# Negai-98/LDT

Measured on AMD Instinct MI355X. Metric: shapes/sec (2048-pt, 1000-step SDE sample), higher is better.
Workload: dtype bf16

## Files before the change

### ldt_amd/csrc/attn_tile.h

```cpp
#pragma once
#include "kernels.h"

template <int DH>
struct AttnLaneOffs {
    int k0;
    int v[DH / 32];
    __device__ __forceinline__ void init(int lane) {
        constexpr int ROWB = DH * 2;
        const int r = lane & 31, hh = lane >> 5;
        const int swk = (DH == 64) ? ((r >> 1) & 7) : ((r >> 2) & 3);
        k0 = r * ROWB + ((hh ^ swk) << 4);
        const int tg = lane >> 4, ti = lane & 15, tq = ti >> 2, tp = ti & 3;
        const int v_row_off = 4 * (tg >> 1) + tq;
        const int v_chunk = (tg & 1) * 2 + (tp >> 1);
        const int v_byte = (tp & 1) * 8;
        const int swv = (DH == 64) ? (((v_row_off >> 1) & 1) << 2) : 0;
#pragma unroll
        for (int d = 0; d < DH / 32; ++d) v[d] = v_row_off * ROWB + (((d * 4 + v_chunk) ^ swv) << 4) + v_byte;
    }
};

#define ATT_THR 6.0f
#ifndef ATT_SCALAR_SOFTMAX
#define ATT_SCALAR_SOFTMAX 0
#endif
template <int DH>
__device__ __forceinline__ void attn_block(const char* Kt, const char* Vt, const int kt, const bf16x8 (&qf)[DH / 16], f32x16 (&oacc)[DH / 32],
                                           float& m_run, float& l_run, int kv0, int Nk, int hh, float c,
                                           const AttnLaneOffs<DH>& lo) {
    constexpr int ROWB = DH * 2, ND = DH / 32, NS = DH / 16;
    {
        f32x16 sacc;
#pragma unroll
        for (int i = 0; i < 16; ++i) sacc[i] = 0.f;
#pragma unroll
        for (int s = 0; s < NS; ++s) {
            const bf16x8 kf = *reinterpret_cast<const bf16x8*>(Kt + kt * 32 * ROWB + (lo.k0 ^ (s << 5)));
            sacc = __builtin_amdgcn_mfma_f32_32x32x16_bf16(kf, qf[s], sacc, 0, 0, 0);
        }
        if (kv0 + kt * 32 + 32 > Nk) {
#pragma unroll
            for (int i = 0; i < 16; ++i) {
                const int key = kv0 + kt * 32 + (i & 3) + 8 * (i >> 2) + 4 * hh;
                sacc[i] = (key < Nk) ? sacc[i] : -INFINITY;
            }
        }
        float mx = __builtin_fmaxf(sacc[0], sacc[1]);
#pragma unroll
        for (int i = 2; i < 16; i += 2) mx = __builtin_fmaxf(__builtin_fmaxf(mx, sacc[i]), sacc[i + 1]);
        mx = fmaxf(mx, __shfl_xor(mx, 32, 64));
        if (__builtin_amdgcn_ballot_w64((mx - m_run) * c > ATT_THR) != 0) {
            const float m_new = fmaxf(m_run, mx);
            const float alpha = __builtin_amdgcn_exp2f((m_run - m_new) * c);
            l_run *= alpha;
            m_run = m_new;
            const f32x2 a2 = {alpha, alpha};
#pragma unroll
            for (int d = 0; d < ND; ++d)
#pragma unroll
                for (int i = 0; i < 16; i += 2) {
                    f32x2 o = {oacc[d][i], oacc[d][i + 1]};
                    o *= a2;
                    oacc[d][i] = o[0]; oacc[d][i + 1] = o[1];
                }
        }
        const f32x2 c2 = {c, c}, nmc2 = {-m_run * c, -m_run * c};
        f32x2 ps2 = {0.f, 0.f};
        bf16x8 pf[2];
#pragma unroll
        for (int i = 0; i < 16; i += 2) {
            const f32x2 sv = {sacc[i], sacc[i + 1]};
            const f32x2 e = sv * c2 + nmc2;
            f32x2 pv;
            pv[0] = __builtin_amdgcn_exp2f(e[0]);
            pv[1] = __builtin_amdgcn_exp2f(e[1]);
            ps2 += pv;
            pf[i >> 3][i & 7] = (bf16_t)pv[0];
            pf[i >> 3][(i & 7) + 1] = (bf16_t)pv[1];
        }
        l_run += ps2[0] + ps2[1];
#pragma unroll
        for (int s2 = 0; s2 < 2; ++s2)
#pragma unroll
            for (int d = 0; d < ND; ++d) {
                const char* base = Vt + (kt * 32 + 16 * s2) * ROWB;
                const bf16x4 v0 = __builtin_amdgcn_ds_read_tr16_b64_v4bf16((__attribute__((address_space(3))) bf16x4*)(base + lo.v[d]));
                const bf16x4 v1 = __builtin_amdgcn_ds_read_tr16_b64_v4bf16((__attribute__((address_space(3))) bf16x4*)(base + 8 * ROWB + lo.v[d]));
                const bf16x8 vf = {v0[0], v0[1], v0[2], v0[3], v1[0], v1[1], v1[2], v1[3]};
                oacc[d] = __builtin_amdgcn_mfma_f32_32x32x16_bf16(vf, pf[s2], oacc[d], 0, 0, 0);
            }
    }
}
template <int DH>
__device__ __forceinline__ void attn_tile(const char* Kt, const char* Vt, const bf16x8 (&qf)[DH / 16], f32x16 (&oacc)[DH / 32],
                                          float& m_run, float& l_run, int kv0, int Nk, int hh, float c,
                                          const AttnLaneOffs<DH>& lo) {
    attn_block<DH>(Kt, Vt, 0, qf, oacc, m_run, l_run, kv0, Nk, hh, c, lo);
    attn_block<DH>(Kt, Vt, 1, qf, oacc, m_run, l_run, kv0, Nk, hh, c, lo);
}

template <int DH>
__device__ __forceinline__ void attn_scores(const char* Kt, const bf16x8 (&qf)[DH / 16], f32x16& s0, f32x16& s1, const AttnLaneOffs<DH>& lo) {
    constexpr int ROWB = DH * 2, NS = DH / 16;
#pragma unroll
    for (int i = 0; i < 16; ++i) { s0[i] = 0.f; s1[i] = 0.f; }
#pragma unroll
    for (int s = 0; s < NS; ++s) {
        const bf16x8 k0 = *reinterpret_cast<const bf16x8*>(Kt + (lo.k0 ^ (s << 5)));
        const bf16x8 k1 = *reinterpret_cast<const bf16x8*>(Kt + 32 * ROWB + (lo.k0 ^ (s << 5)));
        s0 = __builtin_amdgcn_mfma_f32_32x32x16_bf16(k0, qf[s], s0, 0, 0, 0);
        s1 = __builtin_amdgcn_mfma_f32_32x32x16_bf16(k1, qf[s], s1, 0, 0, 0);
    }
}
template <int DH>
__device__ __forceinline__ void attn_softmax_pv(const char* Vt, f32x16& s0, f32x16& s1, f32x16 (&oacc)[DH / 32], float& m_run, float& l_run,
                                                int kv0, int Nk, int hh, float c, const AttnLaneOffs<DH>& lo) {
    constexpr int ROWB = DH * 2, ND = DH / 32;
    if (kv0 + 64 > Nk) {
#pragma unroll
        for (int i = 0; i < 16; ++i) {
            const int key = kv0 + (i & 3) + 8 * (i >> 2) + 4 * hh;
            s0[i] = (key < Nk) ? s0[i] : -INFINITY;
            s1[i] = (key + 32 < Nk) ? s1[i] : -INFINITY;
        }
    }
    float mx = __builtin_fmaxf(s0[0], s1[0]);
#pragma unroll
    for (int i = 1; i < 16; ++i) mx = __builtin_fmaxf(__builtin_fmaxf(mx, s0[i]), s1[i]);
    mx = fmaxf(mx, __shfl_xor(mx, 32, 64));
    if (__builtin_amdgcn_ballot_w64((mx - m_run) * c > ATT_THR) != 0) {
        const float m_new = fmaxf(m_run, mx);
        const float alpha = __builtin_amdgcn_exp2f((m_run - m_new) * c);
        l_run *= alpha;
        m_run = m_new;
        const f32x2 a2 = {alpha, alpha};
#pragma unroll
        for (int d = 0; d < ND; ++d)
#pragma unroll
            for (int i = 0; i < 16; i += 2) {
                f32x2 o = {oacc[d][i], oacc[d][i + 1]};
                o *= a2;
                oacc[d][i] = o[0]; oacc[d][i + 1] = o[1];
            }
    }
    bf16x8 pf[4];
#if ATT_SCALAR_SOFTMAX
    const float nmc = -m_run * c;
    float q0 = 0.f, q1 = 0.f, q2 = 0.f, q3 = 0.f;
#pragma unroll
    for (int i = 0; i < 16; i += 2) {
        float ea0 = __builtin_fmaf(s0[i], c, nmc), ea1 = __builtin_fmaf(s0[i + 1], c, nmc);
        float eb0 = __builtin_fmaf(s1[i], c, nmc), eb1 = __builtin_fmaf(s1[i + 1], c, nmc);
        asm volatile("" : "+v"(ea0), "+v"(ea1), "+v"(eb0), "+v"(eb1));
        const float pa0 = __builtin_amdgcn_exp2f(ea0), pa1 = __builtin_amdgcn_exp2f(ea1);
        const float pb0 = __builtin_amdgcn_exp2f(eb0), pb1 = __builtin_amdgcn_exp2f(eb1);
        q0 += pa0; q1 += pa1; q2 += pb0; q3 += pb1;
        asm volatile("" : "+v"(q0), "+v"(q1), "+v"(q2), "+v"(q3));
        pf[i >> 3][i & 7] = (bf16_t)pa0;       pf[i >> 3][(i & 7) + 1] = (bf16_t)pa1;
        pf[2 + (i >> 3)][i & 7] = (bf16_t)pb0; pf[2 + (i >> 3)][(i & 7) + 1] = (bf16_t)pb1;
    }
    l_run += (q0 + q1) + (q2 + q3);
#else
    const f32x2 c2 = {c, c}, nmc2 = {-m_run * c, -m_run * c};
    f32x2 psa = {0.f, 0.f}, psb = {0.f, 0.f};
#pragma unroll
    for (int i = 0; i < 16; i += 2) {
        const f32x2 ea = (f32x2){s0[i], s0[i + 1]} * c2 + nmc2;
        const f32x2 eb = (f32x2){s1[i], s1[i + 1]} * c2 + nmc2;
        f32x2 pa, pb;
        pa[0] = __builtin_amdgcn_exp2f(ea[0]); pa[1] = __builtin_amdgcn_exp2f(ea[1]);
        pb[0] = __builtin_amdgcn_exp2f(eb[0]); pb[1] = __builtin_amdgcn_exp2f(eb[1]);
        psa += pa; psb += pb;
        pf[i >> 3][i & 7] = (bf16_t)pa[0];       pf[i >> 3][(i & 7) + 1] = (bf16_t)pa[1];
        pf[2 + (i >> 3)][i & 7] = (bf16_t)pb[0]; pf[2 + (i >> 3)][(i & 7) + 1] = (bf16_t)pb[1];
    }
    l_run += (psa[0] + psa[1]) + (psb[0] + psb[1]);
#endif
#pragma unroll
    for (int s2 = 0; s2 < 4; ++s2)
#pragma unroll
        for (int d = 0; d < ND; ++d) {
            const char* base = Vt + 16 * s2 * ROWB;
            const bf16x4 v0 = __builtin_amdgcn_ds_read_tr16_b64_v4bf16((__attribute__((address_space(3))) bf16x4*)(base + lo.v[d]));
            const bf16x4 v1 = __builtin_amdgcn_ds_read_tr16_b64_v4bf16((__attribute__((address_space(3))) bf16x4*)(base + 8 * ROWB + lo.v[d]));
            const bf16x8 vf = {v0[0], v0[1], v0[2], v0[3], v1[0], v1[1], v1[2], v1[3]};
            oacc[d] = __builtin_amdgcn_mfma_f32_32x32x16_bf16(vf, pf[s2], oacc[d], 0, 0, 0);
        }
}

template <int DH>
__device__ __forceinline__ void attn_head_pipelined(const char* Ks, const char* Vs, int ntl, const bf16x8 (&qf)[DH / 16], f32x16 (&oacc)[DH / 32],
                                                    float& m_run, float& l_run, int Nk, int hh, float c, const AttnLaneOffs<DH>& lo) {
    constexpr int TILE = 64 * DH * 2;
    f32x16 sa0, sa1, sb0, sb1;
    attn_scores<DH>(Ks, qf, sa0, sa1, lo);
    int t = 0;
    for (; t + 2 <= ntl; t += 2) {
        attn_scores<DH>(Ks + (t + 1) * TILE, qf, sb0, sb1, lo);
        __builtin_amdgcn_sched_barrier(0);
        attn_softmax_pv<DH>(Vs + t * TILE, sa0, sa1, oacc, m_run, l_run, t * 64, Nk, hh, c, lo);
        __builtin_amdgcn_sched_barrier(0);
        if (t + 2 < ntl) attn_scores<DH>(Ks + (t + 2) * TILE, qf, sa0, sa1, lo);
        __builtin_amdgcn_sched_barrier(0);
        attn_softmax_pv<DH>(Vs + (t + 1) * TILE, sb0, sb1, oacc, m_run, l_run, (t + 1) * 64, Nk, hh, c, lo);
        __builtin_amdgcn_sched_barrier(0);
    }
    if (t < ntl) attn_softmax_pv<DH>(Vs + t * TILE, sa0, sa1, oacc, m_run, l_run, t * 64, Nk, hh, c, lo);
}

template <int DH>
__device__ __forceinline__ void attn_tile_joint(const char* Kt, const char* Vt, const bf16x8 (&qf)[DH / 16], f32x16 (&oacc)[DH / 32],
                                                float& m_run, float& l_run, int kv0, int Nk, int hh, float c,
                                                const AttnLaneOffs<DH>& lo) {
    f32x16 s0, s1;
    attn_scores<DH>(Kt, qf, s0, s1, lo);
    attn_softmax_pv<DH>(Vt, s0, s1, oacc, m_run, l_run, kv0, Nk, hh, c, lo);
}
```

### ldt_amd/csrc/gemm_bf16.hip

```cpp
#include <stdlib.h>

#include <map>
#include <mutex>
#include <tuple>
#include <type_traits>

#include "kernels.h"

#define BK 64

enum { FOLD_NONE = 0, FOLD_PRODUCER = 1, FOLD_CONSUMER = 2 };

template <int ROWS, int NW = 4>
__device__ __forceinline__ void stage_tile(const bf16_t* __restrict__ g, long ld, int row0, int nrows_total,
                                           int k0, char* lds_tile, int wave, int lane) {
#pragma unroll
    for (int p = 0; p < ROWS / (8 * NW); ++p) {
        const int piece = wave * (ROWS / (8 * NW)) + p;
        const int r = piece * 8 + (lane >> 3);
        const int cdst = lane & 7;
        const int csrc = cdst ^ ((r >> 1) & 7);
        int grow = row0 + r;
        grow = grow < nrows_total ? grow : nrows_total - 1;
        const bf16_t* src = g + (long)grow * ld + k0 + csrc * 8;
// ... 543 lines not shown
        auto ktile = [&](auto flags_c) {
            constexpr int FL = decltype(flags_c)::value;
            constexpr bool SKIP = V3_PREISSUE && (FL & KT_FIRST);
            const char* st = smem2 + (gk & 1) * V3_BUF_BYTES;
            char* nb = smem2 + ((gk + 1) & 1) * V3_BUF_BYTES;
            bf16x8 wf[4], xf[4];
            if (!WREG) {
#pragma unroll
                for (int i = 0; i < 4; ++i) wf[i] = *reinterpret_cast<const bf16x8*>(st + wb0 + i * 2048);
            }
#pragma unroll
            for (int i = 0; i < 4; ++i) xf[i] = *reinterpret_cast<const bf16x8*>(st + xb0 + i * 2048);
#if V3_SCHED == 1
            issue_w(nb, 0, 2);
#else
            if (WREG) wload_h1();
            else if (!SKIP) issue_w(nb);
#endif
            if (FL & KT_FOLD_DMA) {
                if (wave < 2 * a.stats_parts) {
                    const float* src = a.stats_in + ((long)(wave >> 1) * a.M + m0 + (wave & 1) * 128) * 2 + lane * 4;
                    __builtin_amdgcn_global_load_lds((const __attribute__((address_space(1))) void*)src,
                                                     (__attribute__((address_space(3))) void*)(stage_reg + V2_STATS_OFF), 16, 0, 0);
                }
                if (wave < 4 && lane < 32) {
                    const float* src = (wave < 2 ? fold_S : fold_C) + n0 + (wave & 1) * 128 + lane * 4;
                    __builtin_amdgcn_global_load_lds((const __attribute__((address_space(1))) void*)src,
                                                     (__attribute__((address_space(3))) void*)(stage_reg + V2_SC_OFF), 16, 0, 0);
                }
            }
            if ((FL & KT_FOLD_FINAL) && wave < 4) v2_fold_finalize(smem2 + V2_RING_BYTES, tid, a.stats_parts, a.K);
            constexpr int P0W = WREG ? (SKIP ? 8 : 4) : SKIP ? 8 : V3_SCHED == 1 ? 2 : 4;
            constexpr bool AFTER_EPI = (FL & KT_FIRST) || (V3_PREISSUE && !WREG && (FL & KT_SECOND));
            if (AFTER_EPI && prev_staged) asm volatile("s_waitcnt vmcnt(%0)" ::"n"(P0W + EPI_VMEM > 63 ? 63 : P0W + EPI_VMEM) : "memory");
            else asm volatile("s_waitcnt vmcnt(%0)" ::"n"(P0W) : "memory");
            V2_BARRIER();
            if (WREG) {
                asm volatile("" : "+v"(w0[0]), "+v"(w0[1]), "+v"(w0[2]), "+v"(w0[3]));
#pragma unroll
                for (int i = 0; i < 4; ++i) wf[i] = __builtin_bit_cast(bf16x8, w0[i]);
            }
            __builtin_amdgcn_s_setprio(1);
#pragma unroll
            for (int ni = 0; ni < 4; ++ni)
#pragma unroll
                for (int mi = 0; mi < 4; ++mi)
                    acc[ni][mi] = __builtin_amdgcn_mfma_f32_16x16x32_bf16(wf[ni], xf[mi], acc[ni][mi], 0, 0, 0);
            __builtin_amdgcn_s_setprio(0);
            V2_BARRIER();
#pragma unroll
            for (int i = 0; i < 4; ++i) xf[i] = *reinterpret_cast<const bf16x8*>(st + xb0 + (4 + i) * 2048);
#if V3_SCHED == 1
            issue_w(nb, 2, 4);
#else
            if (!SKIP) issue_xa(nb);
#endif
            V2_BARRIER();
            __builtin_amdgcn_s_setprio(1);
#pragma unroll
            for (int ni = 0; ni < 4; ++ni)
#pragma unroll
                for (int mi = 0; mi < 4; ++mi)
                    acc[ni][4 + mi] = __builtin_amdgcn_mfma_f32_16x16x32_bf16(wf[ni], xf[mi], acc[ni][4 + mi], 0, 0, 0);
            __builtin_amdgcn_s_setprio(0);
            V2_BARRIER();
            if (!WREG) {
#pragma unroll
                for (int i = 0; i < 4; ++i) wf[i] = *reinterpret_cast<const bf16x8*>(st + wb1 + i * 2048);
            }
#pragma unroll
            for (int i = 0; i < 4; ++i) xf[i] = *reinterpret_cast<const bf16x8*>(st + xb1 + i * 2048);
#if V3_SCHED == 1
            issue_xa(nb);
#else
            if (!SKIP) { issue_xb(nb); advance(); }
#endif
            if (WREG) {
                wload_h0();
                if (SKIP) asm volatile("s_waitcnt vmcnt(4)" ::: "memory");
                else asm volatile("s_waitcnt vmcnt(8)" ::: "memory");
            }
            V2_BARRIER();
            if (WREG) {
                asm volatile("" : "+v"(w1[0]), "+v"(w1[1]), "+v"(w1[2]), "+v"(w1[3]));
#pragma unroll
                for (int i = 0; i < 4; ++i) wf[i] = __builtin_bit_cast(bf16x8, w1[i]);
            }
            __builtin_amdgcn_s_setprio(1);
#pragma unroll
            for (int ni = 0; ni < 4; ++ni)
#pragma unroll
                for (int mi = 0; mi < 4; ++mi)
                    acc[ni][mi] = __builtin_amdgcn_mfma_f32_16x16x32_bf16(wf[ni], xf[mi], acc[ni][mi], 0, 0, 0);
            __builtin_amdgcn_s_setprio(0);
            V2_BARRIER();
#pragma unroll
            for (int i = 0; i < 4; ++i) xf[i] = *reinterpret_cast<const bf16x8*>(st + xb1 + (4 + i) * 2048);
#if V3_SCHED == 1
            issue_xb(nb);
            advance();
#endif
            constexpr int P3W = WREG ? (SKIP ? 4 : 6) : 2;
            if (!WREG && SKIP && prev_staged) asm volatile("s_waitcnt vmcnt(%0)" ::"n"(2 + EPI_VMEM > 63 ? 63 : 2 + EPI_VMEM) : "memory");
            else asm volatile("s_waitcnt vmcnt(%0)" ::"n"(P3W) : "memory");
            V2_BARRIER();
            __builtin_amdgcn_s_setprio(1);
#pragma unroll
            for (int ni = 0; ni < 4; ++ni)
#pragma unroll
                for (int mi = 0; mi < 4; ++mi)
                    acc[ni][4 + mi] = __builtin_amdgcn_mfma_f32_16x16x32_bf16(wf[ni], xf[mi], acc[ni][4 + mi], 0, 0, 0);
            __builtin_amdgcn_s_setprio(0);
            V2_BARRIER();
            ++gk;
        };
#define KTL(f) std::integral_constant<int, (f)>{}
        if (FOLD == FOLD_CONSUMER) {
            ktile(KTL(KT_FIRST)); ktile(KTL(KT_FOLD_DMA | KT_SECOND)); ktile(KTL(KT_PLAIN)); ktile(KTL(KT_FOLD_FINAL));
            for (int kt = 4; kt < nkt; ++kt) ktile(KTL(KT_PLAIN));
        } else {
            ktile(KTL(KT_FIRST)); ktile(KTL(KT_SECOND));
            for (int kt = 2; kt < nkt; ++kt) ktile(KTL(KT_PLAIN));
        }
#undef KTL
        if (grp == 0) V2_BARRIER();

        prev_staged = true;
#if V3_PREISSUE
        if (!XRING) {
            char* pb = smem2 + ((gk + 1) & 1) * V3_BUF_BYTES;
            if (!WREG) issue_w(pb);
            issue_xa(pb); issue_xb(pb); advance();
        }
#endif
        if (XRING) {
            asm volatile("s_waitcnt vmcnt(0)" ::: "memory");
            V2_BARRIER();
            v2_epilogue_staged<EPI, FOLD, 1>(a, acc, m0, n0, grp, wn, lane, lrow, lchk, gate, stage_reg, smem2 + V2_RING_BYTES, ln_scale,
                                                true, g4_pre, sc4_pre, smem2 + wave * 16384);
#if V3_XRING_BREAK
            break;
#else
            if (WREG) break;
#endif
        } else
            v2_epilogue_staged<EPI, FOLD>(a, acc, m0, n0, grp, wn, lane, lrow, lchk, gate, stage_reg, smem2 + V2_RING_BYTES, ln_scale,
                                          it == 0 && (pre_ok || FOLD == FOLD_PRODUCER), g4_pre, sc4_pre);
    }
    asm volatile("s_waitcnt vmcnt(0)" ::: "memory");
}

#include "attn_tile.h"
#define QA_W_ROWS 192
template <int FOLD>
__global__ __launch_bounds__(512) void gemm_qkv_attn256_kernel(const GemmArgs a) {
    static_assert(FOLD == FOLD_NONE || FOLD == FOLD_CONSUMER, "qkv+attention: plain or LN-folded consumer");
    extern __shared__ __attribute__((aligned(16))) char smem2[];
    const int tid = threadIdx.x;
    const int lane = tid & 63;
    const int wave = __builtin_amdgcn_readfirstlane(tid >> 6);
    const int grp = wave >> 2, wn = wave & 3;
    const int lrow = lane & 15, lchk = lane >> 4;
    const int nkt = a.K >> 6;
    const int hidden = a.N / 3, heads = hidden / 64;

    const int tiles_n = heads;
    const int tiles_m = a.M / 256;
    const int tiles = tiles_m * tiles_n;
    const int G = gridDim.x, bid = blockIdx.x;
    const int nx = G < 8 ? G : 8;
    const int xcd = bid % nx, j = bid / nx;
    const int wpx = (G - xcd + nx - 1) / nx;
    const int c_lo = (int)((long)tiles * xcd / nx), c_hi = (int)((long)tiles * (xcd + 1) / nx);
    const int my_tiles = (c_hi - c_lo - j + wpx - 1) / wpx > 0 ? (c_hi - c_lo - j + wpx - 1) / wpx : 0;
    if (my_tiles == 0) return;
    const int gm = a.group_m;
    auto tile_of = [&](int it, int& m0, int& hd) {
        const int id = c_lo + j + it * wpx;
        if (gm <= 1) { m0 = (id / tiles_n) * 256; hd = id % tiles_n; return; }
        const int per = gm * tiles_n, g = id / per, r = id - g * per;
        const int rows = min(gm, tiles_m - g * gm);
        m0 = (g * gm + r % rows) * 256; hd = r / rows;
    };

    int wvo[3], xavo[2], xbvo[2];
    int wds[3], xads[2], xbds[2];
#pragma unroll
    for (int q = 0; q < 3; ++q) {
        const int pj = wave * 3 + q;
        const int r = pj * 8 + (lane >> 3);
        const int gr = (pj >> 3) * hidden + (r & 63);
        wvo[q] = gr * (int)a.ldw * 2 + (((lane & 7) ^ ((r >> 1) & 7)) << 4);
        wds[q] = V3_OPER_BYTES + pj * 1024;
    }
#pragma unroll
    for (int q = 0; q < 2; ++q) {
        const int pj = wave * 2 + q;
        const int r0 = pj < 8 ? pj * 8 : 128 + (pj - 8) * 8;
        const int ra = r0 + (lane >> 3), rb = ra + 64;
        xavo[q] = ra * (int)a.ldx * 2 + (((lane & 7) ^ ((ra >> 1) & 7)) << 4);
        xbvo[q] = rb * (int)a.ldx * 2 + (((lane & 7) ^ ((rb >> 1) & 7)) << 4);
        xads[q] = r0 * 128;
        xbds[q] = (r0 + 64) * 128;
    }
    const char* sxb = nullptr;
    const char* swb = nullptr;
    int s_it = 0, s_kt = 0, s_inc = 128;
    auto seek = [&](int it) {
        int m0, hd;
        tile_of(it, m0, hd);
        sxb = reinterpret_cast<const char*>(a.X + (long)m0 * a.ldx);
        swb = reinterpret_cast<const char*>(a.W + (long)hd * 64 * a.ldw);
    };
    auto advance = [&]() {
        sxb += s_inc; swb += s_inc;
        if (++s_kt == nkt) {
            s_kt = 0;
            if (++s_it < my_tiles) seek(s_it);
            else { sxb -= s_inc; swb -= s_inc; s_inc = 0; s_kt = -0x40000000; }
        }
    };
    int gk = 0;
    auto issue_w = [&](char* buf) {
#pragma unroll
        for (int q = 0; q < 3; ++q)
            __builtin_amdgcn_global_load_lds((const __attribute__((address_space(1))) void*)(swb + wvo[q]),
                                             (__attribute__((address_space(3))) void*)(buf + wds[q]), 16, 0, 0);
    };
    auto issue_xa = [&](char* buf) {
#pragma unroll
        for (int q = 0; q < 2; ++q)
            __builtin_amdgcn_global_load_lds((const __attribute__((address_space(1))) void*)(sxb + xavo[q]),
                                             (__attribute__((address_space(3))) void*)(buf + xads[q]), 16, 0, 0);
    };
    auto issue_xb = [&](char* buf) {
#pragma unroll
        for (int q = 0; q < 2; ++q)
            __builtin_amdgcn_global_load_lds((const __attribute__((address_space(1))) void*)(sxb + xbvo[q]),
                                             (__attribute__((address_space(3))) void*)(buf + xbds[q]), 16, 0, 0);
    };
    seek(0);
    const int step = ((FOLD != FOLD_NONE) && a.step_ptr) ? *a.step_ptr : 0;
    const float* fold_S = (FOLD == FOLD_CONSUMER) ? a.fold_S + (long)step * a.fold_step_stride : nullptr;
    const float* fold_C = (FOLD == FOLD_CONSUMER) ? a.fold_C + (long)step * a.fold_step_stride : nullptr;

    issue_w(smem2); issue_xa(smem2); issue_xb(smem2); advance();
    asm volatile("s_waitcnt vmcnt(2)" ::: "memory");
    V2_BARRIER();

    const int sw = (lrow >> 1) & 7;
    const int xrb = (grp * 128 + lrow) * 128, wrb = V3_OPER_BYTES + (wn * 48 + lrow) * 128;
    const int xb0 = xrb + ((lchk ^ sw) << 4), xb1 = xrb + (((4 + lchk) ^ sw) << 4);
    const int wb0 = wrb + ((lchk ^ sw) << 4), wb1 = wrb + (((4 + lchk) ^ sw) << 4);
    constexpr int EPI_VMEM = 4;
    bool prev_staged = false;
    const int r32 = lane & 31, hh = lane >> 5;
    AttnLaneOffs<64> lo;
    lo.init(lane);

    for (int it = 0; it < my_tiles; ++it) {
        int m0, hd;
        tile_of(it, m0, hd);
        f32x4 acc[3][8];
#pragma unroll
        for (int i = 0; i < 3; ++i)
#pragma unroll
            for (int jj = 0; jj < 8; ++jj) acc[i][jj] = (f32x4){0.f, 0.f, 0.f, 0.f};
        f32x4 add4[3];
#pragma unroll
        for (int ni = 0; ni < 3; ++ni) {
            const int c = wn * 48 + ni * 16 + lchk * 4;
            add4[ni] = (FOLD == FOLD_NONE && a.bias) ? *reinterpret_cast<const f32x4*>(a.bias + (c >> 6) * hidden + hd * 64 + (c & 63)) : (f32x4){0.f, 0.f, 0.f, 0.f};
        }
        if (grp == 1) V2_BARRIER();

        enum { KT_PLAIN = 0, KT_FIRST = 1, KT_FOLD_DMA = 4, KT_FOLD_FINAL = 8 };
        auto ktile = [&](auto flags_c) {
            constexpr int FL = decltype(flags_c)::value;
            const char* st = smem2 + (gk & 1) * V3_BUF_BYTES;
            char* nb = smem2 + ((gk + 1) & 1) * V3_BUF_BYTES;
            bf16x8 wf[3], xf[4];
#pragma unroll
            for (int i = 0; i < 3; ++i) wf[i] = *reinterpret_cast<const bf16x8*>(st + wb0 + i * 2048);
#pragma unroll
            for (int i = 0; i < 4; ++i) xf[i] = *reinterpret_cast<const bf16x8*>(st + xb0 + i * 2048);
            issue_w(nb);
            if (FL & KT_FOLD_DMA) {
                char* stage_reg = smem2 + V2_RING_BYTES + wave * 4096;
                if (wave < 2 * a.stats_parts) {
                    const float* src = a.stats_in + ((long)(wave >> 1) * a.M + m0 + (wave & 1) * 128) * 2 + lane * 4;
                    __builtin_amdgcn_global_load_lds((const __attribute__((address_space(1))) void*)src,
                                                     (__attribute__((address_space(3))) void*)(stage_reg + V2_STATS_OFF), 16, 0, 0);
                }
                if (wave < 6 && lane < 16) {
                    const int seg = wave < 3 ? wave : wave - 3;
                    const float* src = (wave < 3 ? fold_S : fold_C) + seg * hidden + hd * 64 + lane * 4;
                    __builtin_amdgcn_global_load_lds((const __attribute__((address_space(1))) void*)src,
                                                     (__attribute__((address_space(3))) void*)(stage_reg + V2_SC_OFF), 16, 0, 0);
                }
            }
            if ((FL & KT_FOLD_FINAL) && wave < 4) v2_fold_finalize(smem2 + V2_RING_BYTES, tid, a.stats_parts, a.K);
            constexpr int P0W = 3;
            if ((FL & KT_FIRST) && prev_staged) asm volatile("s_waitcnt vmcnt(%0)" ::"n"(P0W + EPI_VMEM) : "memory");
            else asm volatile("s_waitcnt vmcnt(%0)" ::"n"(P0W) : "memory");
            V2_BARRIER();
            __builtin_amdgcn_s_setprio(1);
#pragma unroll
            for (int ni = 0; ni < 3; ++ni)
#pragma unroll
                for (int mi = 0; mi < 4; ++mi)
                    acc[ni][mi] = __builtin_amdgcn_mfma_f32_16x16x32_bf16(wf[ni], xf[mi], acc[ni][mi], 0, 0, 0);
            __builtin_amdgcn_s_setprio(0);
            V2_BARRIER();
#pragma unroll
            for (int i = 0; i < 4; ++i) xf[i] = *reinterpret_cast<const bf16x8*>(st + xb0 + (4 + i) * 2048);
            issue_xa(nb);
            V2_BARRIER();
            __builtin_amdgcn_s_setprio(1);
#pragma unroll
            for (int ni = 0; ni < 3; ++ni)
#pragma unroll
                for (int mi = 0; mi < 4; ++mi)
                    acc[ni][4 + mi] = __builtin_amdgcn_mfma_f32_16x16x32_bf16(wf[ni], xf[mi], acc[ni][4 + mi], 0, 0, 0);
            __builtin_amdgcn_s_setprio(0);
            V2_BARRIER();
#pragma unroll
            for (int i = 0; i < 3; ++i) wf[i] = *reinterpret_cast<const bf16x8*>(st + wb1 + i * 2048);
#pragma unroll
            for (int i = 0; i < 4; ++i) xf[i] = *reinterpret_cast<const bf16x8*>(st + xb1 + i * 2048);
            issue_xb(nb); advance();
            V2_BARRIER();
            __builtin_amdgcn_s_setprio(1);
#pragma unroll
            for (int ni = 0; ni < 3; ++ni)
#pragma unroll
                for (int mi = 0; mi < 4; ++mi)
                    acc[ni][mi] = __builtin_amdgcn_mfma_f32_16x16x32_bf16(wf[ni], xf[mi], acc[ni][mi], 0, 0, 0);
            __builtin_amdgcn_s_setprio(0);
            V2_BARRIER();
#pragma unroll
            for (int i = 0; i < 4; ++i) xf[i] = *reinterpret_cast<const bf16x8*>(st + xb1 + (4 + i) * 2048);
            asm volatile("s_waitcnt vmcnt(2)" ::: "memory");
            V2_BARRIER();
            __builtin_amdgcn_s_setprio(1);
#pragma unroll
            for (int ni = 0; ni < 3; ++ni)
#pragma unroll
                for (int mi = 0; mi < 4; ++mi)
                    acc[ni][4 + mi] = __builtin_amdgcn_mfma_f32_16x16x32_bf16(wf[ni], xf[mi], acc[ni][4 + mi], 0, 0, 0);
            __builtin_amdgcn_s_setprio(0);
            V2_BARRIER();
            ++gk;
        };
#define KTL(f) std::integral_constant<int, (f)>{}
        if (FOLD == FOLD_CONSUMER) {
            ktile(KTL(KT_FIRST)); ktile(KTL(KT_FOLD_DMA)); ktile(KTL(KT_PLAIN)); ktile(KTL(KT_FOLD_FINAL));
            for (int kt = 4; kt < nkt; ++kt) ktile(KTL(KT_PLAIN));
        } else {
            ktile(KTL(KT_FIRST));
            for (int kt = 1; kt < nkt; ++kt) ktile(KTL(KT_PLAIN));
        }
#undef KTL
        if (grp == 0) V2_BARRIER();
        prev_staged = true;

        char* stage_base = smem2 + V2_RING_BYTES;
        char* kvb = smem2 + ((gk + 1) & 1) * V3_BUF_BYTES;
        f32x4 s4[3];
        float rr[8], nm[8];
        if (FOLD == FOLD_CONSUMER) {
#pragma unroll
            for (int mi = 0; mi < 8; ++mi) {
                const int R = grp * 128 + mi * 16 + lrow;
                const f32x2 t = *reinterpret_cast<const f32x2*>(stage_base + (R >> 7) * 4096 + V2_STATS_OFF + (R & 127) * 8);
                rr[mi] = t[0]; nm[mi] = t[1];
            }
#pragma unroll
            for (int ni = 0; ni < 3; ++ni) {
                const int c = wn * 48 + ni * 16 + lchk * 4;
                s4[ni] = *reinterpret_cast<const f32x4*>(stage_base + (c >> 6) * 4096 + V2_SC_OFF + (c & 63) * 4);
                add4[ni] = *reinterpret_cast<const f32x4*>(stage_base + (3 + (c >> 6)) * 4096 + V2_SC_OFF + (c & 63) * 4);
            }
            asm volatile("s_waitcnt lgkmcnt(0)" ::: "memory");
            V2_BARRIER();
        }
#pragma unroll
        for (int mi = 0; mi < 8; ++mi) {
            const int R = grp * 128 + mi * 16 + lrow;
            const int swr = (R >> 1) & 7;
#pragma unroll
            for (int ni = 0; ni < 3; ++ni) {
                f32x4 v = acc[ni][mi];
                if (FOLD == FOLD_CONSUMER) {
#pragma unroll
                    for (int r = 0; r < 4; ++r) v[r] = v[r] * rr[mi] + (nm[mi] * s4[ni][r] + add4[ni][r]);
                } else {
#pragma unroll
                    for (int r = 0; r < 4; ++r) v[r] += add4[ni][r];
                }
                const bf16x4 pk = {(bf16_t)v[0], (bf16_t)v[1], (bf16_t)v[2], (bf16_t)v[3]};
                const int c = wn * 48 + ni * 16 + lchk * 4, seg = c >> 6, cc = c & 63;
                const int sz = seg == 2 ? ((R >> 1) & 1) << 2 : swr;
                char* dst = (seg == 0 ? stage_base : kvb + (seg - 1) * 32768) + R * 128 + (((cc >> 3) ^ sz) << 4) + (cc & 7) * 2;
                *reinterpret_cast<bf16x4*>(dst) = pk;
            }
        }
        asm volatile("s_waitcnt lgkmcnt(0)" ::: "memory");
        V2_BARRIER();

        {
            const int q0 = wave * 32;
            bf16x8 qf[4];
#pragma unroll
            for (int sI = 0; sI < 4; ++sI)
                qf[sI] = *reinterpret_cast<const bf16x8*>(stage_base + (q0 + r32) * 128 + (((hh + 2 * sI) ^ ((r32 >> 1) & 7)) << 4));
            f32x16 oacc[2];
#pragma unroll
            for (int d = 0; d < 2; ++d)
#pragma unroll
                for (int i = 0; i < 16; ++i) oacc[d][i] = 0.f;
            float m_run = -INFINITY, l_run = 0.f;
            f32x16 sa0, sa1, sb0, sb1;
            const char* Kt = kvb;
            const char* Vt = kvb + 32768;
            const float csc = a.attn_scale_log2e;
            attn_scores<64>(Kt, qf, sa0, sa1, lo);
            __builtin_amdgcn_sched_barrier(0);
            attn_scores<64>(Kt + 8192, qf, sb0, sb1, lo);
            __builtin_amdgcn_sched_barrier(0);
            attn_softmax_pv<64>(Vt, sa0, sa1, oacc, m_run, l_run, 0, 256, hh, csc, lo);
            __builtin_amdgcn_sched_barrier(0);
            attn_scores<64>(Kt + 2 * 8192, qf, sa0, sa1, lo);
            __builtin_amdgcn_sched_barrier(0);
            attn_softmax_pv<64>(Vt + 8192, sb0, sb1, oacc, m_run, l_run, 64, 256, hh, csc, lo);
            __builtin_amdgcn_sched_barrier(0);
            attn_scores<64>(Kt + 3 * 8192, qf, sb0, sb1, lo);
            __builtin_amdgcn_sched_barrier(0);
            attn_softmax_pv<64>(Vt + 2 * 8192, sa0, sa1, oacc, m_run, l_run, 128, 256, hh, csc, lo);
            __builtin_amdgcn_sched_barrier(0);
            attn_softmax_pv<64>(Vt + 3 * 8192, sb0, sb1, oacc, m_run, l_run, 192, 256, hh, csc, lo);
            char* ost = stage_base + q0 * 128;
            const float inv = 1.0f / (l_run + __shfl_xor(l_run, 32, 64));
#pragma unroll
            for (int d = 0; d < 2; ++d)
#pragma unroll
                for (int g = 0; g < 4; ++g) {
                    const int chn = d * 4 + g;
                    const bf16x4 pk = {(bf16_t)(oacc[d][4 * g + 0] * inv), (bf16_t)(oacc[d][4 * g + 1] * inv),
                                       (bf16_t)(oacc[d][4 * g + 2] * inv), (bf16_t)(oacc[d][4 * g + 3] * inv)};
                    *reinterpret_cast<bf16x4*>(ost + r32 * 128 + ((chn ^ (r32 & 7)) << 4) + hh * 8) = pk;
                }
            asm volatile("s_waitcnt lgkmcnt(0)" ::: "memory");
            bf16_t* ob = a.attn_o + (((long)(m0 >> 8) * heads + hd) * 256 + q0) * 64;
#pragma unroll
            for (int p4 = 0; p4 < 4; ++p4) {
                const int row = p4 * 8 + (lane >> 3), ch = lane & 7;
                const bf16x8 v = *reinterpret_cast<const bf16x8*>(ost + row * 128 + ((ch ^ (row & 7)) << 4));
                *reinterpret_cast<bf16x8*>(ob + (long)row * 64 + ch * 8) = v;
            }
        }
        asm volatile("s_waitcnt lgkmcnt(0)" ::: "memory");
        V2_BARRIER();
    }
    asm volatile("s_waitcnt vmcnt(0)" ::: "memory");
}

__global__ __launch_bounds__(256) void pack_wfrag_kernel(const bf16_t* __restrict__ W, long ldw, int N, int K, bf16_t* __restrict__ Wp) {
    const long c = (long)blockIdx.x * 256 + threadIdx.x;
    const int nkt = K >> 6;
    if (c >= (long)N * K / 8) return;
    const int lane = (int)(c & 63), f = (int)((c >> 6) & 7);
    const long t = c >> 9;
    const int kt = (int)(t % nkt), n64 = (int)(t / nkt);
    const int n = n64 * 64 + (f & 3) * 16 + (lane & 15), k = kt * 64 + (f >> 2) * 32 + (lane >> 4) * 8;
    *reinterpret_cast<bf16x8*>(Wp + c * 8) = *reinterpret_cast<const bf16x8*>(W + (long)n * ldw + k);
}
int ldt_gemm_pack_wfrag_launch(const bf16_t* W, long ldw, int N, int K, bf16_t* Wp, hipStream_t stream) {
    LDT_REQUIRE(W && Wp && N > 0 && K > 0 && N % 64 == 0 && K % 64 == 0 && ldw >= K && ldw % 8 == 0 && ldt_aligned16(W) && ldt_aligned16(Wp), LDT_ESHAPE,
                "pack_wfrag: N=%d and K=%d must be multiples of 64, rows 16-byte aligned (ldw=%ld)", N, K, ldw);
    const long chunks = (long)N * K / 8;
    hipLaunchKernelGGL(pack_wfrag_kernel, dim3((unsigned)((chunks + 255) / 256)), dim3(256), 0, stream, W, ldw, N, K, Wp);
    return ldt_check_launch("pack_wfrag");
}
static std::atomic<int> g_dbg_wreg{-1};
extern "C" int ldt_dbg_gemm_wreg(int32_t on) { g_dbg_wreg.store(on); return LDT_OK; }
static const bf16_t* dbg_wfrag_cached(const bf16_t* W, long ldw, int N, int K, hipStream_t stream) {
    static std::mutex mu;
    static std::map<std::tuple<const void*, long, int, int>, bf16_t*> cache;
    std::lock_guard<std::mutex> lk(mu);
    auto key = std::make_tuple((const void*)W, ldw, N, K);
    auto itc = cache.find(key);
    if (itc != cache.end()) return itc->second;
    bf16_t* wp = nullptr;
    if (hipMalloc((void**)&wp, (size_t)N * K * 2) != hipSuccess) return nullptr;
    if (ldt_gemm_pack_wfrag_launch(W, ldw, N, K, wp, stream) != LDT_OK) { (void)hipFree(wp); return nullptr; }
    cache[key] = wp;
    return wp;
}

static std::atomic<int> g_group_m{-1};
extern "C" int ldt_dbg_gemm_group_m(int32_t gm) { g_group_m.store(gm); return LDT_OK; }
static std::atomic<int> g_dbg_epi{-1};
extern "C" int ldt_dbg_gemm_epi(int32_t bits) { g_dbg_epi.store(bits); return LDT_OK; }

static bool gemm256_takes(int epi, const GemmArgs* a) {
    return a->K % 64 == 0 && a->K >= 128 && a->M % 256 == 0 && a->N % 256 == 0 && a->ldo % 8 == 0 &&
           (epi != EPI_RESID_F32 || (a->ldr % 4 == 0 && (!a->gate || a->gate_sample_stride % 4 == 0))) &&
           (epi != EPI_RELU_BF16 || !a->skip || a->lds_ % 4 == 0);
}

template <int EPI, int FOLD = FOLD_NONE>
static int launch_256(const GemmArgs* a_in, hipStream_t stream) {
    static const int gm_env = getenv("LDT_GEMM_GM") ? atoi(getenv("LDT_GEMM_GM")) : -1;
    const int gm_dbg = g_group_m.load();
    GemmArgs a_copy = *a_in;
    const int tn = a_in->N / 256, tm = a_in->M / 256;
    a_copy.group_m = gm_dbg >= 0 ? gm_dbg : gm_env >= 0 ? gm_env : (tn >= 8 && tm >= 8) ? 4 : 1;
    static const bool xring_on = !(getenv("LDT_RESID_RING") && atoi(getenv("LDT_RESID_RING")) == 0);
    const bool xring = (EPI == EPI_RESID_F32 && xring_on && a_in->resid && ldt_aligned16(a_in->resid) && (!a_in->gate || a_in->gate_sample_stride == 0));
    static const int dbg_env = getenv("LDT_DBG_EPI") ? atoi(getenv("LDT_DBG_EPI")) : 0;
    a_copy.dbg = g_dbg_epi.load() >= 0 ? g_dbg_epi.load() : dbg_env;
    const GemmArgs* a = &a_copy;
    LDT_REQUIRE(gemm256_takes(EPI, a), LDT_ESHAPE, "gemm256: M=%d N=%d must be multiples of 256, K=%d of 64 (>= 128), rows 16-byte aligned", a->M, a->N, a->K);
    constexpr bool WREG_BUILT = (EPI == EPI_RESID_F32) && V3_PREISSUE == 1 && V3_SCHED == 0;
    static const int wreg_env = getenv("LDT_GEMM_WREG") ? atoi(getenv("LDT_GEMM_WREG")) : -1;
    const int wreg_dbg = g_dbg_wreg.load() >= 0 ? g_dbg_wreg.load() : wreg_env;
    const int tiles = tm * tn;
    static const int cap = getenv("LDT_GEMM_GRID") ? atoi(getenv("LDT_GEMM_GRID")) : LDT_NUM_CUS;
    const int lim = (a->max_wgs > 0 && a->max_wgs < cap) ? a->max_wgs : cap;
    const int grid = tiles < lim ? tiles : lim;
    if constexpr (EPI == EPI_RESID_F32) {
        if (xring && grid == tiles && a->dbg == 0) {
            if (WREG_BUILT && wreg_dbg == 1 && !a_copy.Wp) a_copy.Wp = dbg_wfrag_cached(a->W, a->ldw, a->N, a->K, stream);
            const bool wreg = WREG_BUILT && a_copy.Wp && wreg_dbg != 0 && ldt_aligned16(a_copy.Wp);
            const bool klong = a->K >= 2048;
#define LAUNCH_XR(W, KL)                                                                                                          \
    do {                                                                                                                          \
        LDT_ENSURE_LDS((&gemm_bf16_nt_256f_kernel<EPI, FOLD, 1, W, KL>), V2_LDS_BYTES, "gemm256f");                                \
        hipLaunchKernelGGL((gemm_bf16_nt_256f_kernel<EPI, FOLD, 1, W, KL>), dim3(grid), dim3(512), V2_LDS_BYTES, stream, *a);     \
    } while (0)
            if constexpr (WREG_BUILT) {
                if (wreg) {
                    if (klong) LAUNCH_XR(1, 1); else LAUNCH_XR(1, 0);
                    return ldt_check_launch("gemm_bf16_nt_256f");
                }
            }
            if (klong) LAUNCH_XR(0, 1); else LAUNCH_XR(0, 0);
#undef LAUNCH_XR
            return ldt_check_launch("gemm_bf16_nt_256f");
        }
    }
    LDT_ENSURE_LDS((&gemm_bf16_nt_256f_kernel<EPI, FOLD>), V2_LDS_BYTES, "gemm256f");
    hipLaunchKernelGGL((gemm_bf16_nt_256f_kernel<EPI, FOLD>), dim3(grid), dim3(512), V2_LDS_BYTES, stream, *a);
    return ldt_check_launch("gemm_bf16_nt_256f");
}

static int gemm_variant_env();
bool ldt_gemm_qkv_attn256_try(const GemmArgs* a_in, int tokens, int head_dim, bool folded, hipStream_t stream, int* status) {
    static const bool on = !(getenv("LDT_QKV_ATTN256") && atoi(getenv("LDT_QKV_ATTN256")) == 0);
    const GemmArgs& g = *a_in;
    if (!on || gemm_variant_env() != 0 || tokens != 256 || head_dim != 64 || !g.attn_o) return false;
    if (g.N % 192 != 0 || (g.N / 3) % 64 != 0 || g.M % 256 != 0 || g.K % 64 != 0 || g.K < (folded ? 256 : 128)) return false;
    if (folded && (g.stats_parts <= 0 || g.stats_parts > 4 || g.stats_parts * 256 != g.K || !g.stats_in || !g.fold_S || !g.fold_C ||
                   !ldt_aligned16(g.stats_in) || !ldt_aligned16(g.fold_S) || !ldt_aligned16(g.fold_C) || g.fold_step_stride % 4 != 0))
        return false;
    if (!ldt_aligned16(g.X) || !ldt_aligned16(g.W) || !ldt_aligned16(g.attn_o) || (g.bias && !ldt_aligned16(g.bias)) || g.ldx % 8 != 0 || g.ldw % 8 != 0 ||
        g.ldx < g.K || g.ldw < g.K)
        return false;
    const int tm = g.M / 256, tn = (g.N / 3) / 64;
    const long tiles = (long)tm * tn;
    const int lim = (g.max_wgs > 0 && g.max_wgs < LDT_NUM_CUS) ? g.max_wgs : LDT_NUM_CUS;
    if (tiles * 8 < (long)lim * 5) return false;
    GemmArgs a = g;
    static const int gm_env = getenv("LDT_QKV_GM") ? atoi(getenv("LDT_QKV_GM")) : getenv("LDT_GEMM_GM") ? atoi(getenv("LDT_GEMM_GM")) : -1;
    a.group_m = gm_env >= 0 ? gm_env : (tn >= 8 && tm >= 8) ? 4 : 1;
    const int grid = tiles < lim ? (int)tiles : lim;
    auto launch = [&]() -> int {
        if (folded) {
            LDT_ENSURE_LDS((&gemm_qkv_attn256_kernel<FOLD_CONSUMER>), V2_LDS_BYTES, "gemm_qkv_attn256");
            hipLaunchKernelGGL((gemm_qkv_attn256_kernel<FOLD_CONSUMER>), dim3(grid), dim3(512), V2_LDS_BYTES, stream, a);
        } else {
            LDT_ENSURE_LDS((&gemm_qkv_attn256_kernel<FOLD_NONE>), V2_LDS_BYTES, "gemm_qkv_attn256");
            hipLaunchKernelGGL((gemm_qkv_attn256_kernel<FOLD_NONE>), dim3(grid), dim3(512), V2_LDS_BYTES, stream, a);
        }
        return ldt_check_launch("gemm_qkv_attn256");
    };
    *status = launch();
    return true;
}

static int gemm_variant_env() {
    static int v = -1;
    if (v < 0) { const char* e = getenv("LDT_GEMM_FORCE"); v = e ? atoi(e) : 0; }
    return v;
}
bool ldt_gemm_lnfold_v1_route(int M, int D, int F, int max_wgs) {
    const int lim = (max_wgs > 0 && max_wgs < LDT_NUM_CUS) ? max_wgs : LDT_NUM_CUS;
    auto small = [&](int N) { return (long)((M + 255) / 256) * ((N + 255) / 256) * 8 < (long)lim * 5; };
    if (!(gemm_variant_env() == 0 && M % 128 == 0 && D % 64 == 0 && F % 64 == 0 && D <= 1024 && small(D) && small(3 * D) && small(F))) return false;
    if ((long)(M / 64) * (D / 128) * 8 < (long)lim * 5) return false;
    return ldt_gemm_mid_lnfold_takes(EPI_RESID_F32, M, D, D) && ldt_gemm_mid_lnfold_takes(EPI_RESID_F32, M, D, F) &&
           ldt_gemm_mid_lnfold_takes(EPI_BF16, M, 3 * D, D) && ldt_gemm_mid_lnfold_takes(EPI_GELU_BF16, M, F, D);
}

int ldt_gemm_lnfold_launch(int epi, const GemmArgs* a, hipStream_t stream) {
    const int width = epi == EPI_RESID_F32 ? a->N : a->K;
    const bool v1 = a->stats_parts > 0 && a->stats_parts * 32 == width && a->stats_parts * 256 != width;
    if (v1) LDT_REQUIRE(a->M > 0 && a->M % 128 == 0 && a->N % 64 == 0 && a->K >= 128 && a->K % BK == 0, LDT_ESHAPE,
                        "gemm_lnfold (v1 route): M=%d must be a multiple of 128, N=%d of 64, K=%d >= 128, K %% 64 == 0", a->M, a->N, a->K);
    else LDT_REQUIRE(a->M > 0 && a->N > 0 && a->K >= 256 && a->M % 256 == 0 && a->N % 256 == 0 && a->K % BK == 0, LDT_ESHAPE,
                     "gemm_lnfold: M=%d N=%d must be multiples of 256 and K=%d >= 256, K %% 64 == 0", a->M, a->N, a->K);
    LDT_REQUIRE(a->ldx % 8 == 0 && a->ldw % 8 == 0 && a->ldx >= a->K && a->ldw >= a->K && a->ldo % 8 == 0 && ldt_aligned16(a->X) &&
                ldt_aligned16(a->W) && ldt_aligned16(a->out), LDT_EALIGN, "gemm_lnfold: operands must be 16-byte aligned (ldx=%ld ldw=%ld ldo=%ld)",
                a->ldx, a->ldw, a->ldo);
    if (epi == EPI_RESID_F32) {
        LDT_REQUIRE(a->resid && a->ldr % 4 == 0 && ldt_aligned16(a->resid), LDT_EALIGN, "gemm_lnfold: resid missing/misaligned");
        LDT_REQUIRE(!a->gate || (a->rows_per_sample > 0 && ldt_aligned16(a->gate) && a->gate_sample_stride % 4 == 0 && a->gate_step_stride % 4 == 0),
// ... 103 lines not shown
```

Measured before the change: 6.469.

## Add extra V-tile LDS swizzle and hoist first-k-tile MFMA ahead of fold DMA

Adds an optional second XOR swizzle on V rows in LDS, applied both where the QKV epilogue writes V and where the transposed reads fetch it, with the second half-read XORed by 32. The goal is fewer LDS bank conflicts in the ds_read_tr loads for the PV product. The first k-tile's wait, barrier and MFMA block and the next X fragment loads are also moved ahead of the fold-stats DMA issue, so that DMA overlaps compute. Timestamp instrumentation is added behind a compile-time flag that is off by default.

Result: faster. 6.547, median of 6 (+1.2%).

```diff
diff --git a/ldt_amd/csrc/attn_tile.h b/ldt_amd/csrc/attn_tile.h
--- a/ldt_amd/csrc/attn_tile.h
+++ b/ldt_amd/csrc/attn_tile.h
@@ -1,7 +1,7 @@
 #pragma once
 #include "kernels.h"
 
-template <int DH>
+template <int DH, int VSW = 0>
 struct AttnLaneOffs {
     int k0;
     int v[DH / 32];
@@ -16,7 +16,7 @@
         const int v_byte = (tp & 1) * 8;
         const int swv = (DH == 64) ? (((v_row_off >> 1) & 1) << 2) : 0;
 #pragma unroll
-        for (int d = 0; d < DH / 32; ++d) v[d] = v_row_off * ROWB + (((d * 4 + v_chunk) ^ swv) << 4) + v_byte;
+        for (int d = 0; d < DH / 32; ++d) v[d] = v_row_off * ROWB + (((d * 4 + v_chunk) ^ swv ^ (VSW ? (v_row_off >> 2) & 3 : 0)) << 4) + v_byte;
     }
 };
 
@@ -99,8 +99,8 @@
     attn_block<DH>(Kt, Vt, 1, qf, oacc, m_run, l_run, kv0, Nk, hh, c, lo);
 }
 
-template <int DH>
-__device__ __forceinline__ void attn_scores(const char* Kt, const bf16x8 (&qf)[DH / 16], f32x16& s0, f32x16& s1, const AttnLaneOffs<DH>& lo) {
+template <int DH, int VSW = 0>
+__device__ __forceinline__ void attn_scores(const char* Kt, const bf16x8 (&qf)[DH / 16], f32x16& s0, f32x16& s1, const AttnLaneOffs<DH, VSW>& lo) {
     constexpr int ROWB = DH * 2, NS = DH / 16;
 #pragma unroll
     for (int i = 0; i < 16; ++i) { s0[i] = 0.f; s1[i] = 0.f; }
@@ -112,9 +112,9 @@
         s1 = __builtin_amdgcn_mfma_f32_32x32x16_bf16(k1, qf[s], s1, 0, 0, 0);
     }
 }
-template <int DH>
+template <int DH, int VSW = 0>
 __device__ __forceinline__ void attn_softmax_pv(const char* Vt, f32x16& s0, f32x16& s1, f32x16 (&oacc)[DH / 32], float& m_run, float& l_run,
-                                                int kv0, int Nk, int hh, float c, const AttnLaneOffs<DH>& lo) {
+                                                int kv0, int Nk, int hh, float c, const AttnLaneOffs<DH, VSW>& lo) {
     constexpr int ROWB = DH * 2, ND = DH / 32;
     if (kv0 + 64 > Nk) {
 #pragma unroll
@@ -182,7 +182,7 @@
         for (int d = 0; d < ND; ++d) {
             const char* base = Vt + 16 * s2 * ROWB;
             const bf16x4 v0 = __builtin_amdgcn_ds_read_tr16_b64_v4bf16((__attribute__((address_space(3))) bf16x4*)(base + lo.v[d]));
-            const bf16x4 v1 = __builtin_amdgcn_ds_read_tr16_b64_v4bf16((__attribute__((address_space(3))) bf16x4*)(base + 8 * ROWB + lo.v[d]));
+            const bf16x4 v1 = __builtin_amdgcn_ds_read_tr16_b64_v4bf16((__attribute__((address_space(3))) bf16x4*)(base + 8 * ROWB + (VSW ? lo.v[d] ^ 32 : lo.v[d])));
             const bf16x8 vf = {v0[0], v0[1], v0[2], v0[3], v1[0], v1[1], v1[2], v1[3]};
             oacc[d] = __builtin_amdgcn_mfma_f32_32x32x16_bf16(vf, pf[s2], oacc[d], 0, 0, 0);
         }
diff --git a/ldt_amd/csrc/gemm_bf16.hip b/ldt_amd/csrc/gemm_bf16.hip
--- a/ldt_amd/csrc/gemm_bf16.hip
+++ b/ldt_amd/csrc/gemm_bf16.hip
@@ -719,6 +719,14 @@
 
 #include "attn_tile.h"
 #define QA_W_ROWS 192
+#ifdef QA_STAMPS
+__device__ long long* g_qa_stamps;
+extern "C" int ldt_dbg_qa_stamps(void* p) { return (int)hipMemcpyToSymbol(HIP_SYMBOL(g_qa_stamps), &p, sizeof(p)); }
+#define QA_STAMP_AT(idx) do { const long long _t = __builtin_amdgcn_s_memtime(); _stv = (lane == (idx)) ? _t : _stv; } while (0)
+#define QA_STAMP(sec) do { if (it < 4) QA_STAMP_AT(it * 12 + (sec)); } while (0)
+#else
+#define QA_STAMP(sec)
+#endif
 template <int FOLD>
 __global__ __launch_bounds__(512) void gemm_qkv_attn256_kernel(const GemmArgs a) {
     static_assert(FOLD == FOLD_NONE || FOLD == FOLD_CONSUMER, "qkv+attention: plain or LN-folded consumer");
@@ -822,12 +830,18 @@
     constexpr int EPI_VMEM = 4;
     bool prev_staged = false;
     const int r32 = lane & 31, hh = lane >> 5;
-    AttnLaneOffs<64> lo;
+    AttnLaneOffs<64, 1> lo;
     lo.init(lane);
+#ifdef QA_STAMPS
+    long long _stv = 0;
+    QA_STAMP_AT(56);
+    { const long long _r = __builtin_amdgcn_s_memrealtime(); _stv = (lane == 57) ? _r : _stv; }
+#endif
 
     for (int it = 0; it < my_tiles; ++it) {
         int m0, hd;
         tile_of(it, m0, hd);
+        QA_STAMP(0);
         f32x4 acc[3][8];
 #pragma unroll
         for (int i = 0; i < 3; ++i)
@@ -852,6 +866,22 @@
 #pragma unroll
             for (int i = 0; i < 4; ++i) xf[i] = *reinterpret_cast<const bf16x8*>(st + xb0 + i * 2048);
             issue_w(nb);
+            if ((FL & KT_FOLD_FINAL) && wave < 4) v2_fold_finalize(smem2 + V2_RING_BYTES, tid, a.stats_parts, a.K);
+            constexpr int P0W = 3;
+            if ((FL & KT_FIRST) && prev_staged) asm volatile("s_waitcnt vmcnt(%0)" ::"n"(P0W + EPI_VMEM) : "memory");
+            else asm volatile("s_waitcnt vmcnt(%0)" ::"n"(P0W) : "memory");
+            V2_BARRIER();
+            __builtin_amdgcn_s_setprio(1);
+#pragma unroll
+            for (int ni = 0; ni < 3; ++ni)
+#pragma unroll
+                for (int mi = 0; mi < 4; ++mi)
+                    acc[ni][mi] = __builtin_amdgcn_mfma_f32_16x16x32_bf16(wf[ni], xf[mi], acc[ni][mi], 0, 0, 0);
+            __builtin_amdgcn_s_setprio(0);
+            V2_BARRIER();
+#pragma unroll
+            for (int i = 0; i < 4; ++i) xf[i] = *reinterpret_cast<const bf16x8*>(st + xb0 + (4 + i) * 2048);
+            issue_xa(nb);
             if (FL & KT_FOLD_DMA) {
                 char* stage_reg = smem2 + V2_RING_BYTES + wave * 4096;
                 if (wave < 2 * a.stats_parts) {
@@ -866,22 +896,6 @@
                                                      (__attribute__((address_space(3))) void*)(stage_reg + V2_SC_OFF), 16, 0, 0);
                 }
             }
-            if ((FL & KT_FOLD_FINAL) && wave < 4) v2_fold_finalize(smem2 + V2_RING_BYTES, tid, a.stats_parts, a.K);
-            constexpr int P0W = 3;
-            if ((FL & KT_FIRST) && prev_staged) asm volatile("s_waitcnt vmcnt(%0)" ::"n"(P0W + EPI_VMEM) : "memory");
-            else asm volatile("s_waitcnt vmcnt(%0)" ::"n"(P0W) : "memory");
-            V2_BARRIER();
-            __builtin_amdgcn_s_setprio(1);
-#pragma unroll
-            for (int ni = 0; ni < 3; ++ni)
-#pragma unroll
-                for (int mi = 0; mi < 4; ++mi)
-                    acc[ni][mi] = __builtin_amdgcn_mfma_f32_16x16x32_bf16(wf[ni], xf[mi], acc[ni][mi], 0, 0, 0);
-            __builtin_amdgcn_s_setprio(0);
-            V2_BARRIER();
-#pragma unroll
-            for (int i = 0; i < 4; ++i) xf[i] = *reinterpret_cast<const bf16x8*>(st + xb0 + (4 + i) * 2048);
-            issue_xa(nb);
             V2_BARRIER();
             __builtin_amdgcn_s_setprio(1);
 #pragma unroll
@@ -921,15 +935,19 @@
         };
 #define KTL(f) std::integral_constant<int, (f)>{}
         if (FOLD == FOLD_CONSUMER) {
-            ktile(KTL(KT_FIRST)); ktile(KTL(KT_FOLD_DMA)); ktile(KTL(KT_PLAIN)); ktile(KTL(KT_FOLD_FINAL));
+            ktile(KTL(KT_FIRST)); QA_STAMP(1);
+            ktile(KTL(KT_FOLD_DMA)); QA_STAMP(2);
+            ktile(KTL(KT_PLAIN)); ktile(KTL(KT_FOLD_FINAL));
             for (int kt = 4; kt < nkt; ++kt) ktile(KTL(KT_PLAIN));
         } else {
-            ktile(KTL(KT_FIRST));
-            for (int kt = 1; kt < nkt; ++kt) ktile(KTL(KT_PLAIN));
+            ktile(KTL(KT_FIRST)); QA_STAMP(1);
+            for (int kt = 1; kt < nkt; ++kt) { ktile(KTL(KT_PLAIN)); if (kt == 1) QA_STAMP(2); }
         }
 #undef KTL
+        QA_STAMP(3);
         if (grp == 0) V2_BARRIER();
         prev_staged = true;
+        QA_STAMP(4);
 
         char* stage_base = smem2 + V2_RING_BYTES;
         char* kvb = smem2 + ((gk + 1) & 1) * V3_BUF_BYTES;
@@ -967,13 +985,14 @@
                 }
                 const bf16x4 pk = {(bf16_t)v[0], (bf16_t)v[1], (bf16_t)v[2], (bf16_t)v[3]};
                 const int c = wn * 48 + ni * 16 + lchk * 4, seg = c >> 6, cc = c & 63;
-                const int sz = seg == 2 ? ((R >> 1) & 1) << 2 : swr;
+                const int sz = seg == 2 ? (((R >> 1) & 1) << 2) | ((R >> 2) & 3) : swr;
                 char* dst = (seg == 0 ? stage_base : kvb + (seg - 1) * 32768) + R * 128 + (((cc >> 3) ^ sz) << 4) + (cc & 7) * 2;
                 *reinterpret_cast<bf16x4*>(dst) = pk;
             }
         }
         asm volatile("s_waitcnt lgkmcnt(0)" ::: "memory");
         V2_BARRIER();
+        QA_STAMP(5);
 
         {
             const int q0 = wave * 32;
@@ -993,10 +1012,12 @@
             const float csc = a.attn_scale_log2e;
             attn_scores<64>(Kt, qf, sa0, sa1, lo);
             __builtin_amdgcn_sched_barrier(0);
+            QA_STAMP(6);
             attn_scores<64>(Kt + 8192, qf, sb0, sb1, lo);
             __builtin_amdgcn_sched_barrier(0);
             attn_softmax_pv<64>(Vt, sa0, sa1, oacc, m_run, l_run, 0, 256, hh, csc, lo);
             __builtin_amdgcn_sched_barrier(0);
+            QA_STAMP(7);
             attn_scores<64>(Kt + 2 * 8192, qf, sa0, sa1, lo);
             __builtin_amdgcn_sched_barrier(0);
             attn_softmax_pv<64>(Vt + 8192, sb0, sb1, oacc, m_run, l_run, 64, 256, hh, csc, lo);
@@ -1006,6 +1027,10 @@
             attn_softmax_pv<64>(Vt + 2 * 8192, sa0, sa1, oacc, m_run, l_run, 128, 256, hh, csc, lo);
             __builtin_amdgcn_sched_barrier(0);
             attn_softmax_pv<64>(Vt + 3 * 8192, sb0, sb1, oacc, m_run, l_run, 192, 256, hh, csc, lo);
+#ifdef QA_STAMPS
+            asm volatile("s_nop 0" :: "v"(oacc[0][0]), "v"(oacc[1][0]));
+            QA_STAMP(8);
+#endif
             char* ost = stage_base + q0 * 128;
             const float inv = 1.0f / (l_run + __shfl_xor(l_run, 32, 64));
 #pragma unroll
@@ -1025,11 +1050,22 @@
                 const bf16x8 v = *reinterpret_cast<const bf16x8*>(ost + row * 128 + ((ch ^ (row & 7)) << 4));
                 *reinterpret_cast<bf16x8*>(ob + (long)row * 64 + ch * 8) = v;
             }
+            QA_STAMP(9);
         }
         asm volatile("s_waitcnt lgkmcnt(0)" ::: "memory");
         V2_BARRIER();
+        QA_STAMP(10);
     }
     asm volatile("s_waitcnt vmcnt(0)" ::: "memory");
+#ifdef QA_STAMPS
+    QA_STAMP_AT(58);
+    { const long long _r = __builtin_amdgcn_s_memrealtime(); _stv = (lane == 59) ? _r : _stv; }
+    if (g_qa_stamps) {
+        const long long _h = __builtin_amdgcn_s_getreg((4 << 0) | (0 << 6) | (31 << 11));
+        _stv = lane == 62 ? _h : _stv;
+        g_qa_stamps[((long)blockIdx.x * 8 + wave) * 64 + lane] = _stv;
+    }
+#endif
 }
 
 __global__ __launch_bounds__(256) void pack_wfrag_kernel(const bf16_t* __restrict__ W, long ldw, int N, int K, bf16_t* __restrict__ Wp) {
```
